# harvardinformatics/IMCoalHMM

Hardware: AMD Instinct MI355X
Metric: alignment columns/sec (forward pass), 20-state isolation HMM (higher is better)
Workload: dtype f64

## Files before the change

### imcoalhmm_amd/csrc/imcoal_fwd.hip

```cpp
#include <hip/hip_runtime.h>

#include <algorithm>
#include <cerrno>
#include <climits>
#include <cmath>
#include <cstdint>
#include <cstdio>
#include <cstdlib>
#include <cstring>
#include <list>
#include <atomic>
#include <chrono>
#include <map>
#include <set>
#include <memory>
#include <mutex>
#include <condition_variable>
#include <string>
#include <vector>

#include <unistd.h>

#include "../../include/imcoal_fwd.h"
#include "kernels_plain.hpp"
// ... 82 lines not shown
    uint64_t next_obs_id = 1, next_dict_id = 1;
    size_t seg_override = 0;
    int compression = 1;
    int kernel_pref = 0;
    bool profile = false;
    bool rank1_handoff = true;
    int blocked_variant = 4;
    int wide_blocked = -1;
    int z4_stream = -1;
    bool table_pairs = true;
    int table_triples = -1;
    bool table_split = true;
    int table_split_max = -1;
    bool xcd_affine = true;
    int fuse_tail = 1;
    bool fuse_head = true;
    bool pack_table = true;
    bool guard = false;
    bool use_graphs = false;
    std::vector<Ev3> events;
    std::map<int, std::shared_ptr<DictDev>> dicts;
    uint64_t last_plan[8] = {0, 0, 0, 0, 0, 0, 0, 0};
    uint64_t r1_checked = 0, r1_collapsed = 0;
    std::string last_kernels;
    std::vector<const void *> lds_opted;
} g;

void drop_plans();
void model_release();

// ... 19 lines not shown
    if (std::strncmp(prop.gcnArchName, "gfx950", 6) != 0)
        return fail(IMC_ERR_NODEVICE, std::string("device is ") + prop.gcnArchName + ", this library is built for gfx950 only");
    g.cus = prop.multiProcessorCount > 0 ? prop.multiProcessorCount : 256;
    HIP_TRY(hipStreamCreateWithFlags(&g.stream, hipStreamNonBlocking));
    g.use_graphs = std::getenv("IMC_GRAPH") != nullptr;
    if (const char *gd = std::getenv("IMC_GUARD")) g.guard = std::atoi(gd) != 0;
    if (const char *bv = std::getenv("IMC_BLOCKED")) { const int v = std::atoi(bv); if (v >= 2 && v <= 5) g.blocked_variant = v; }
    if (const char *r1 = std::getenv("IMC_RANK1")) g.rank1_handoff = std::atoi(r1) != 0;
    if (const char *pt = std::getenv("IMC_PACK_TABLE")) g.pack_table = std::atoi(pt) != 0;
    if (const char *tp = std::getenv("IMC_TABLE_PAIRS")) g.table_pairs = std::atoi(tp) != 0;
    if (const char *fh = std::getenv("IMC_FUSE_HEAD")) g.fuse_head = std::atoi(fh) != 0;
    if (const char *ts = std::getenv("IMC_TABLE_SPLIT")) g.table_split = std::atoi(ts) != 0;
    if (const char *tm = std::getenv("IMC_TABLE_SPLIT_MAX")) g.table_split_max = std::max(0, std::atoi(tm));
    if (const char *tt = std::getenv("IMC_TABLE_TRIPLES")) g.table_triples = std::atoi(tt) != 0 ? 1 : 0;
    if (const char *ft = std::getenv("IMC_FUSE_TAIL")) g.fuse_tail = std::max(0, std::min(2, std::atoi(ft)));
    if (const char *xa = std::getenv("IMC_XCD_AFFINE")) g.xcd_affine = std::atoi(xa) != 0;
    if (const char *wb = std::getenv("IMC_WIDE_BLOCKED")) { const int v = std::atoi(wb); if (v >= -1 && v <= 1) g.wide_blocked = v; }
    if (const char *zs = std::getenv("IMC_Z4_STREAM")) { const int v = std::atoi(zs); if (v >= -1 && v <= 1) g.z4_stream = v; }
    g.pid = me;
    g.ready = true;
    return IMC_OK;
}

struct GuardRec { hipDeviceptr_t va; size_t va_size; hipMemGenericAllocationHandle_t handle; hipDeviceptr_t map; size_t map_size; };
std::map<void *, GuardRec> &g_guard = *new std::map<void *, GuardRec>();

hipError_t dev_alloc(void **p, size_t bytes)
{
    bytes = std::max<size_t>(bytes, 16);
    if (!g.guard) return hipMalloc(p, bytes);
// ... 224 lines not shown
    if (zipped) {
        if (int rc = install_encoding(o, dd, enc)) {
            obs_release(o);
            delete o;
            return rc;
        }
    }
    *out = o;
    return IMC_OK;
}


using ChainFn = void (*)(const ChainDesc *, int, const uint32_t *, uint32_t, uint32_t, const double *, const int *,
                         const int *, uint32_t, double *, int *, double *, int);

struct KernelChoice {
    int R = 0, G = 0, NP = 0, VPW = 0, minw = 1;
    void (*plain)(PropArgs) = nullptr;
    void (*zip)(PropArgs) = nullptr;
    size_t (*zip_lds)(int) = nullptr;
    ChainFn chain = nullptr;
    void (*big_table_raw)(BigArgs) = nullptr;
    void (*big_table_level)(BigArgs, const uint16_t *, int) = nullptr;
    void (*big_prop)(BigArgs, const BigBlock *) = nullptr;
    int big_prop_waves = 0;
    void (*big_vec)(BigArgs, const BigBlock *, int, int) = nullptr;
    void (*big_vec_tail)(BigArgs, const BigBlock *, int, int) = nullptr;
    int big_vec_waves = 0;
    int big_nslab = 0;
    size_t big_lds = 0;
    void (*zip2)(BigArgs) = nullptr;
    size_t (*zip2_lds)(int) = nullptr;
    void (*zip3)(BigArgs) = nullptr;
    size_t (*zip3_lds)(int) = nullptr;
    void (*zip4)(BigArgs) = nullptr;
    void (*zip4w)(BigArgs) = nullptr;
// ... 16 lines not shown
    bool chain_self_emax = false;
    bool use3() const;
    size_t blocked_lds(int A) const { return use3() ? zip3_lds(A) : zip2_lds(A); }
};

template <int R, int G, int MW>
KernelChoice make_kc()
{
    constexpr int NP = R * G;
    KernelChoice k;
    k.R = R; k.G = G; k.NP = NP; k.VPW = 64 / G; k.minw = MW;
    k.plain = k_propagate<R, G, MW>;
    k.zip = k_zpropagate<R, G>;
    k.zip_lds = &ZipGeom<R, G>::lds_bytes;
    k.chain = k_chain<NP, (NP <= 12 ? 6 : NP <= 24 ? 4 : NP <= 32 ? 3 : NP <= 64 ? 2 : 1)>;
    k.chain_self_emax = true;
    if constexpr (NP % 4 == 0 && NP <= 24) {
        k.zip2 = k_zpropagate2<NP / 4>;
        k.zip2_lds = &Zip2Geom<NP / 4>::lds_bytes;
        k.zip3 = k_zpropagate3<NP / 4>;
        k.zip3_lds = &Zip3Geom<NP / 4>::lds_bytes;
        k.tok_doubles = Zip3Geom<NP / 4>::TOK;
        if constexpr (NP <= 24) {
            k.zip4 = k_zpropagate4<NP / 4, false, true>;
            k.zip4w = k_zpropagate4<NP / 4, true, true>;
            k.zip4s = k_zpropagate4<NP / 4, false, false>;
            k.zip4sw = k_zpropagate4<NP / 4, true, false>;
            k.zip4_raw = k_z4_raw<NP / 4>;
            k.zip4_level = k_z4_level<NP / 4>;
            k.zip4_level2 = k_z4_level2<NP / 4, false>;
// ... 134 lines not shown

struct Plan {
    std::vector<uint64_t> key;
    KernelChoice *kc = nullptr;
    bool wide = false;
    int N = 0, S = 0, B = 0, n_chunks = 0;
    uint32_t n_segs = 0, n_vecs = 0;
    std::vector<Group> groups;
    size_t pstride = 0;
    SegDesc *d_segs = nullptr;
    VecDesc *d_vecs = nullptr;
    std::vector<Level> levels;
    int32_t *d_final_vec = nullptr;
    uint64_t chain_steps = 0;
    bool finish_fused = false;
    double *d_params = nullptr, *d_out = nullptr;
    double *h_params[2] = {nullptr, nullptr};
    hipEvent_t ev_params[2] = {nullptr, nullptr};
    bool ev_used[2] = {false, false};
    int slot = 0;
    double *h_out = nullptr;
    double *h_out_dev = nullptr;
    double *h_params_dev[2] = {nullptr, nullptr};
    hipStream_t last_stream = nullptr;
    int last_slot = 0;
    bool have_last = false;
    bool busy = false;
    hipGraphExec_t graph = nullptr;
    uint64_t calls = 0;
    uint64_t lp[8] = {0, 0, 0, 0, 0, 0, 0, 0};
    std::string kernels;
    void release()
    {
        if (graph) (void)hipGraphExecDestroy(graph);
        dev_free(d_segs); dev_free(d_vecs); dev_free(d_final_vec);
        for (auto &l : levels) l.release();
        for (auto &gr : groups) { dev_free(gr.d_seg_ids); dev_free(gr.d_seg_out); dev_free(gr.d_blocks); dev_free(gr.d_hot); dev_free(gr.d_tab_desc); dev_free(gr.d_tab_desc2); dev_free(gr.d_tab_desc3); dev_free(gr.d_tails); dev_free(gr.d_tailX); dev_free(gr.d_tailE); dev_free(gr.d_tail_arrive); dev_free(gr.d_tab_order); dev_free(gr.d_tab_lvl); dev_free(gr.d_big_blocks); dev_free(gr.d_Ctab); dev_free(gr.d_Cpack); dev_free(gr.d_cex); dev_free(gr.d_tail_blocks); dev_free(gr.d_r1flag); dev_free(gr.d_r1at); dev_free(gr.d_r1u); dev_free(gr.d_r1alpha); }
        dev_free(d_params); dev_free(d_out);
        for (int k = 0; k < 2; ++k) { (void)hipHostFree(h_params[k]); if (ev_params[k]) (void)hipEventDestroy(ev_params[k]); }
        (void)hipHostFree(h_out);
    }
};

std::list<std::unique_ptr<Plan>> g_plans;
constexpr size_t MAX_PLANS = 4;

void wait_all_idle(std::unique_lock<std::mutex> &lk)
{
    g_cv.wait(lk, [] {
        for (auto &p : g_plans)
// ... 85 lines not shown
    int n_chunks = 0, N = 0, S = 0, B = 0;
    bool op_mode = false;
    KernelChoice *kc = nullptr;
    bool wide = false, wide_ok = true;
    bool mfma() const { return kc->use3() || wide; }
    std::unique_ptr<Plan> p;
    bool big = false;
    std::vector<int> chunk_group;
    std::vector<SegDesc> segs;
    std::vector<uint8_t> seg_first;
    std::vector<uint32_t> chunk_seg;
    std::vector<VecDesc> vecs;
    std::vector<std::vector<std::pair<uint32_t, uint32_t>>> chunk_units;
    std::vector<uint32_t> chunk_unit, unit_vec0;
    std::vector<uint8_t> unit_first;
    struct HostLevel { std::vector<uint32_t> chunk_seg, vec0; std::vector<uint8_t> first; std::vector<ChainDesc> chains; uint32_t n_vecs; };
    std::vector<HostLevel> hl;
    std::vector<int32_t> final_vec;

    static bool z4_streamed(double tables_bytes, int n_sets)
    {
        if (g.z4_stream >= 0) return g.z4_stream == 1;
        return (g.xcd_affine && n_sets > 1) || tables_bytes <= Z4_STREAM_MAX_BYTES;
    }

    size_t handoff_head(const Group &gr) const
    {
        double cols = 0.0, toks = 0.0;
        for (int f : gr.chunks) { cols += (double)chunks[f]->L; toks += (double)(gr.zip ? chunks[f]->ntok[gr.level] : chunks[f]->L); }
        const double span = toks > 0.0 ? cols / toks : 1.0;
        return round_up(std::max<size_t>(R1_MIN_HEAD, (size_t)(R1_HEAD_COLUMNS / span)), 16);
    }

// ... 367 lines not shown
                else
                    for (Z2Block &bk : gr.blocks)
                        if (bk.first == 2) bk.first = 1;
            }
        }
        if (vecs.size() >= (size_t)UINT32_MAX / 2) return fail(IMC_ERR_ARG, "too many vectors in one call");
        p->n_segs = (uint32_t)segs.size();
        p->n_vecs = (uint32_t)vecs.size();
        p->pstride = round_up((size_t)kc->NP + (size_t)kc->NP * kc->NP + (size_t)S * kc->NP, 2);

        return IMC_OK;
    }

    void make_hierarchy()
    {
        hl.assign(1, HostLevel());
        hl[0].chunk_seg = chunk_unit; hl[0].vec0 = unit_vec0; hl[0].first = unit_first; hl[0].n_vecs = p->n_vecs;
        for (;;) {
            const HostLevel &cur = hl.back();
            uint32_t kmax = 0;
            for (int f = 0; f < n_chunks; ++f) kmax = std::max(kmax, cur.chunk_seg[f + 1] - cur.chunk_seg[f]);
            if (kmax <= 1 && hl.size() > 1) break;
            if (kmax == 0) break;
            const uint32_t gsz = kmax <= 16 ? kmax : std::max<uint32_t>(12, (uint32_t)std::ceil(std::cbrt((double)kmax)));
            p->chain_steps += gsz;
            HostLevel nx;
            nx.chunk_seg.assign(n_chunks + 1, 0);
            nx.n_vecs = 0;
            for (int f = 0; f < n_chunks; ++f) {
                nx.chunk_seg[f] = (uint32_t)nx.vec0.size();
                const uint32_t s0 = cur.chunk_seg[f], s1 = cur.chunk_seg[f + 1];
                for (uint32_t rb = s0; rb < s1; rb += gsz) {
                    const uint32_t re = std::min(rb + gsz, s1);
                    const bool fst = rb == s0 && !op_mode;
                    nx.vec0.push_back(nx.n_vecs);
                    nx.first.push_back(fst);
                    const int nvv = fst ? 1 : N;
                    for (int c = 0; c < nvv; ++c) nx.chains.push_back(ChainDesc{rb, re, (uint32_t)c, nx.n_vecs + c, fst ? 1u : 0u, 0u});
                    nx.n_vecs += nvv;
                }
            }
            nx.chunk_seg[n_chunks] = (uint32_t)nx.vec0.size();
            const bool done = kmax <= gsz;
            hl.push_back(std::move(nx));
            if (done) break;
        }
        final_vec.assign(std::max(n_chunks, 1), -1);
        bool all_from_chains = hl.size() > 1 && !op_mode && n_chunks > 0;
        for (int f = 0; f < n_chunks; ++f) {
            const HostLevel &last = hl.back();
            if (last.chunk_seg[f + 1] > last.chunk_seg[f]) final_vec[f] = (int32_t)last.vec0[last.chunk_seg[f]];
            else all_from_chains = false;
        }
        p->finish_fused = false;
        if (all_from_chains) {
            HostLevel &last = hl.back();
            std::vector<char> seen((size_t)n_chunks, 0);
            for (ChainDesc &cd : last.chains)
                for (int f = 0; f < n_chunks; ++f)
                    if (cd.first && final_vec[f] == (int32_t)cd.out_vec) { cd.chunk1 = (uint32_t)f + 1; seen[f] = 1; }
            p->finish_fused = std::all_of(seen.begin(), seen.end(), [](char c) { return c != 0; });
            if (!p->finish_fused)
                for (ChainDesc &cd : last.chains) cd.chunk1 = 0;
        }

    }

    int upload(Plan **out)
    {
        while (g_plans.size() >= MAX_PLANS) {
            auto victim = g_plans.end();
            for (auto it = g_plans.begin(); it != g_plans.end(); ++it)
                if (!(*it)->busy) victim = it;
            if (victim == g_plans.end()) break;
            (*victim)->release();
            g_plans.erase(victim);
        }

        Plan *q = p.get();
        auto up = [&](void **d, const void *h, size_t bytes) -> hipError_t {
// ... 12 lines not shown
        if (e == hipSuccess) e = up((void **)&q->d_vecs, vecs.data(), vecs.size() * sizeof(VecDesc));
        if (e == hipSuccess) e = up((void **)&q->d_final_vec, final_vec.data(), final_vec.size() * 4);
        q->levels.resize(hl.size());
        for (size_t l = 0; l < hl.size() && e == hipSuccess; ++l) {
            Level &lv = q->levels[l];
            lv.n_segs = (uint32_t)hl[l].vec0.size();
            lv.n_vecs = hl[l].n_vecs;
            lv.n_chains = (uint32_t)hl[l].chains.size();
            const size_t nv = std::max<size_t>(lv.n_vecs, 1), ns = std::max<size_t>(lv.n_segs, 1);
            e = up((void **)&lv.d_vec0, hl[l].vec0.data(), hl[l].vec0.size() * 4);
            if (e == hipSuccess) e = up((void **)&lv.d_first, hl[l].first.data(), hl[l].first.size());
            if (e == hipSuccess) e = up((void **)&lv.d_chains, hl[l].chains.data(), hl[l].chains.size() * sizeof(ChainDesc));
            if (e == hipSuccess) e = zalloc((void **)&lv.d_P, (size_t)B * nv * kc->NP * 8);
            if (e == hipSuccess) e = zalloc((void **)&lv.d_EX, (size_t)B * nv * 4);
            if (e == hipSuccess) e = zalloc((void **)&lv.d_EMAX, (size_t)B * ns * 4);
        }
        for (Group &gr : q->groups) {
            if (gr.zip2 && e == hipSuccess) e = up((void **)&gr.d_blocks, gr.blocks.data(), gr.blocks.size() * sizeof(Z2Block));
            if (!gr.tails.empty() && e == hipSuccess) {
                const size_t slots = (size_t)B * n_chunks * gr.tail_stride;
                e = up((void **)&gr.d_tails, gr.tails.data(), gr.tails.size() * sizeof(Z2Tail));
                if (e == hipSuccess) e = dev_alloc((void **)&gr.d_tailX, slots * kc->tok_doubles * 8);
                if (e == hipSuccess) e = dev_alloc((void **)&gr.d_tailE, slots * 128);
                if (e == hipSuccess) e = zalloc((void **)&gr.d_tail_arrive, (size_t)B * n_chunks * 4);
            }
            if (gr.zip4 && e == hipSuccess) {
                std::vector<uint64_t> cnt((size_t)gr.A, 0);
                for (int f : gr.chunks)
                    for (size_t z = 0; z < chunks[f]->tok_count[gr.level].size() && z < cnt.size(); ++z) cnt[z] += chunks[f]->tok_count[gr.level][z];
                const std::vector<uint16_t> ids = imc::hot_order(cnt);
// ... 56 lines not shown
        if (e == hipSuccess) e = hipHostGetDevicePointer((void **)&q->h_out_dev, q->h_out, 0);
        if (e != hipSuccess) {
            q->release();
            return fail(e == hipErrorOutOfMemory ? IMC_ERR_OOM : IMC_ERR_HIP,
                        std::string("plan allocation: ") + hipGetErrorString(e));
        }
        g_plans.push_front(std::move(p));
        *out = q;
        return IMC_OK;
    }
};

int build_plan(const imc_obs *const *chunks, int n_chunks, int N, int S, int B, bool op_mode, Plan **out)
{
    std::vector<uint64_t> key;
    key.reserve(n_chunks + 5);
    for (int f = 0; f < n_chunks; ++f) key.push_back(chunks[f]->id);
    key.push_back((uint64_t)N); key.push_back((uint64_t)S); key.push_back((uint64_t)B);
    key.push_back((uint64_t)g.seg_override); key.push_back((uint64_t)(g.compression * 4 + g.kernel_pref + (op_mode ? 64 : 0) + g.blocked_variant * 128 + (g.z4_stream + 1) * 1024 + (g.wide_blocked + 1) * 4096));
    { const char *fl = std::getenv("IMC_FORCE_LEVEL"); key.push_back(fl ? (uint64_t)(std::atoi(fl) + 1) : 0u); }
    for (auto it = g_plans.begin(); it != g_plans.end(); ++it) {
        if ((*it)->key == key) {
            g_plans.splice(g_plans.begin(), g_plans, it);
            *out = g_plans.front().get();
            return IMC_OK;
        }
    }
    bool prefer_gemm = g.kernel_pref == 2;
    if (g.kernel_pref == 0 && N > 24 && N <= 64 && n_chunks > 0) {
        double total = 0.0;
        for (int f = 0; f < n_chunks; ++f) total += (double)chunks[f]->L;
        bool tokens = g.compression != 0;
        for (int f = 0; f < n_chunks; ++f) tokens = tokens && chunks[f]->dict && chunks[f]->nsym == S;
        prefer_gemm = total >= 1.0e6 && total / n_chunks >= 5.0e3 && (tokens || N > 40);
    }
// ... 394 lines not shown
    const size_t lds = ((size_t)WPB * kc->VPW * kc->NP + (size_t)p->S * kc->NP) * 8;
    if (lds > LDS_BUDGET) return fail(IMC_ERR_ARG, "emission table (S x N) too large for LDS");
    if (lds > 48 * 1024)
        if (int rc = allow_lds_budget(kc->plain)) return rc;
    hipLaunchKernelGGL(kc->plain, grid, dim3(WPB * 64), lds, stream, prop_args(p, gr));
    note("k_propagate<" + std::to_string(kc->R) + "," + std::to_string(kc->G) + ">" + stream_tag(gr));
    account(gr);
    HIP_TRY(hipGetLastError());
    return IMC_OK;
}


int Launch::stitch() const
{
    const int N = p->N, NP = kc->NP;
    for (size_t l = 0; l + 1 < p->levels.size(); ++l) {
        const Level &in = p->levels[l], &ot = p->levels[l + 1];
        if (!in.n_segs || !ot.n_chains) continue;
        if (!kc->chain_self_emax) {
            hipLaunchKernelGGL(k_emax, dim3((in.n_segs + 255) / 256, (unsigned)B), dim3(256), 0, stream,
                               in.d_vec0, in.d_first, in.n_segs, in.n_vecs, N, in.d_EX, in.d_EMAX);
            HIP_TRY(hipGetLastError());
        }
        const int threads = (int)round_up((size_t)NP, 64);
        const bool last_level = l + 2 == p->levels.size();
        hipLaunchKernelGGL(kc->chain, dim3(ot.n_chains, (unsigned)B), dim3(threads), 0, stream,
                           ot.d_chains, N, in.d_vec0, in.n_segs, in.n_vecs, in.d_P, in.d_EX, in.d_EMAX,
                           ot.n_vecs, ot.d_P, ot.d_EX, (last_level && p->finish_fused) ? out : (double *)nullptr, p->n_chunks);
        HIP_TRY(hipGetLastError());
    }
    if (p->n_chunks && !p->finish_fused) {
        const Level &last = p->levels.back();
        hipLaunchKernelGGL(k_finish, dim3((p->n_chunks + 63) / 64, (unsigned)B), dim3(64), 0, stream,
                           p->d_final_vec, p->n_chunks, N, NP, last.n_vecs, last.d_P, last.d_EX, out);
        HIP_TRY(hipGetLastError());
    }
    return IMC_OK;
}

int enqueue(Plan *p, hipStream_t stream, double *out, bool allow_tail = true)
{
    hipStreamCaptureStatus cap = hipStreamCaptureStatusNone;
    (void)hipStreamIsCapturing(stream, &cap);
    if (cap == hipStreamCaptureStatusNone && p->have_last && p->last_stream != stream)
        HIP_TRY(hipStreamWaitEvent(stream, p->ev_params[p->last_slot], 0));
// ... 21 lines not shown
    if (L.tail_used) L.note("fused-tail");
    if (!L.tail_used)
        if (int rc = L.stitch()) return rc;
    if (L.prof) {
        HIP_TRY(hipEventRecord(L.ev.c, stream));
        g.events.push_back(L.ev);
    }
    if (cap == hipStreamCaptureStatusNone) {
        HIP_TRY(hipEventRecord(p->ev_params[p->slot], stream));
        p->ev_used[p->slot] = true;
        p->last_stream = stream;
        p->last_slot = p->slot;
        p->have_last = true;
    }
    return IMC_OK;
}

void collect_rank1_stats(Plan *p)
{
    g.r1_checked = g.r1_collapsed = 0;
    for (Group &gr : p->groups) {
        if (!gr.rank1 || gr.r1_segs.empty() || gr.checkpoints.empty()) continue;
        std::vector<int> flags((size_t)p->B * p->n_segs);
        if (hipMemcpy(flags.data(), gr.d_r1flag, flags.size() * 4, hipMemcpyDeviceToHost) != hipSuccess) continue;
        for (int b = 0; b < p->B; ++b)
            for (const auto &sl : gr.r1_segs) {
                if ((int)sl.second <= gr.checkpoints[0]) continue;
                ++g.r1_checked;
                g.r1_collapsed += flags[(size_t)b * p->n_segs + sl.first] ? 1 : 0;
            }
// ... 46 lines not shown
        explicit Busy(Plan *q) : p(q) { p->busy = true; }
        ~Busy() { p->busy = false; g_cv.notify_all(); }
    } busy(p);
    const auto h1 = now();
    if (int rc = stage_params(p, pis, Ts, Es, g.use_graphs)) return rc;
    const size_t n_out = (size_t)B * n_chunks;
    for (size_t k = 0; k < n_out; ++k) reinterpret_cast<volatile uint64_t *>(p->h_out)[k] = OUT_SENTINEL;
    std::atomic_thread_fence(std::memory_order_release);
    const auto h2 = now();
    const bool use_graph = !g.profile && g.use_graphs && p->calls >= 1;
    if (use_graph && !p->graph) {
        hipGraph_t gr = nullptr;
        HIP_TRY(hipStreamBeginCapture(g.stream, hipStreamCaptureModeThreadLocal));
        const int rc = enqueue(p, g.stream, p->h_out_dev);
        const hipError_t ec = hipStreamEndCapture(g.stream, &gr);
        if (rc) { if (gr) (void)hipGraphDestroy(gr); return rc; }
        if (ec != hipSuccess) return fail(IMC_ERR_HIP, std::string("hipStreamEndCapture: ") + hipGetErrorString(ec));
        const hipError_t ei = hipGraphInstantiate(&p->graph, gr, nullptr, nullptr, 0);
        (void)hipGraphDestroy(gr);
        if (ei != hipSuccess) { p->graph = nullptr; return fail(IMC_ERR_HIP, std::string("hipGraphInstantiate: ") + hipGetErrorString(ei)); }
    }
    if (use_graph) HIP_TRY(hipGraphLaunch(p->graph, g.stream));
    else if (int rc = enqueue(p, g.stream, p->h_out_dev)) return rc;
    ++p->calls;
    for (int k = 0; k < 8; ++k) g.last_plan[k] = p->lp[k];
    g.last_kernels = p->kernels;
    const auto h3 = now();
    const hipStream_t st = g.stream;
    lk.unlock();
    const hipError_t ew = n_out ? wait_results(st, p->h_out, n_out) : hipStreamSynchronize(st);
    lk.lock();
    HIP_TRY(ew);
    const auto h4 = now();
    collect_rank1_stats(p);
    if (dbg_host) {
        auto us = [](auto a, auto b) { return std::chrono::duration<double, std::micro>(b - a).count(); };
        static double acc[5] = {0, 0, 0, 0, 0};
        static int n_acc = 0;
        acc[0] += us(h0, h1); acc[1] += us(h1, h2); acc[2] += us(h2, h3); acc[3] += us(h3, h4); acc[4] += us(h4, now());
        if (++n_acc % 20 == 0) {
            fprintf(stderr, "[imc] host us per call: check+plan %.1f  stage %.1f  enqueue %.1f  sync wait %.1f  stats %.1f\n",
                    acc[0] / 20, acc[1] / 20, acc[2] / 20, acc[3] / 20, acc[4] / 20);
            for (double &a : acc) a = 0.0;
        }
    }
    for (int b = 0; b < B; ++b) {
// ... 9 lines not shown
}

int run_state(const imc_obs *const *chunks, int n_chunks, bool op_mode, int B, int N, int S, const double *pis,
              const double *Ts, const double *Es, double *out_state, int *out_exp)
{
    std::lock_guard<std::mutex> lk(g_mu);
    if (int rc = ensure_ctx()) return rc;
    if (int rc = check_args(chunks, n_chunks, B, N, S, pis, Ts, Es)) return rc;
    if (!out_state || !out_exp) return fail(IMC_ERR_ARG, "output buffer is null");
    for (int f = 0; f < n_chunks; ++f)
        if (chunks[f]->L == 0) return fail(IMC_ERR_ARG, "imc_forward_state: empty chunk");
    HIP_TRY(hipSetDevice(g.device));
    Plan *p = nullptr;
    if (int rc = build_plan(chunks, n_chunks, N, S, B, op_mode, &p)) return rc;
    if (int rc = stage_params(p, pis, Ts, Es, g.use_graphs)) return rc;
    if (int rc = enqueue(p, g.stream, p->d_out, false)) return rc;
    ++p->calls;
    for (int k = 0; k < 8; ++k) g.last_plan[k] = p->lp[k];
    g.last_kernels = p->kernels;
    const size_t per = op_mode ? (size_t)N * N : (size_t)N, pere = op_mode ? (size_t)N : 1;
    const size_t n_state = (size_t)B * n_chunks * per, n_exp = (size_t)B * n_chunks * pere;
    double *d_state = nullptr;
    int *d_exp = nullptr;
    hipError_t e = dev_alloc((void **)&d_state, std::max<size_t>(n_state * 8, 16));
    if (e == hipSuccess) e = dev_alloc((void **)&d_exp, std::max<size_t>(n_exp * 4, 16));
    if (e == hipSuccess) {
        const Level &last = p->levels.back();
        hipLaunchKernelGGL(k_export, dim3((unsigned)n_chunks, (unsigned)B), dim3(256), 0, g.stream, p->d_final_vec, n_chunks, N,
                           p->kc->NP, last.n_vecs, last.d_P, last.d_EX, op_mode ? 1 : 0, d_state, d_exp);
        e = hipGetLastError();
    }
// ... 627 lines not shown
    return run_batch(chunks, n_chunks, B, N, S, pis, Ts, Es, nullptr, out_per_chunk);
}

int imc_forward_batch_device(const imc_obs *const *chunks, int n_chunks, int B, int N, int S, const double *pis,
                             const double *Ts, const double *Es, double *d_out_partial, void *hip_stream)
{
    if (!d_out_partial) return fail(IMC_ERR_ARG, "d_out_partial is null");
    std::lock_guard<std::mutex> lk(g_mu);
    if (int rc = ensure_ctx()) return rc;
    if (int rc = check_args(chunks, n_chunks, B, N, S, pis, Ts, Es)) return rc;
    HIP_TRY(hipSetDevice(g.device));
    hipStream_t st = (hipStream_t)hip_stream;
    Plan *p = nullptr;
    if (int rc = build_plan(chunks, n_chunks, N, S, B, false, &p)) return rc;
    if (int rc = stage_params(p, pis, Ts, Es, g.use_graphs)) return rc;
    if (int rc = enqueue(p, st, p->d_out)) return rc;
    ++p->calls;
    for (int k = 0; k < 8; ++k) g.last_plan[k] = p->lp[k];
    g.last_kernels = p->kernels;
    hipLaunchKernelGGL(k_sum_chunks, dim3((B + 63) / 64), dim3(64), 0, st, p->d_out, n_chunks, B, d_out_partial);
    HIP_TRY(hipGetLastError());
    return IMC_OK;
}

int imc_set_segment_length(size_t columns)
{
    std::lock_guard<std::mutex> lk(g_mu);
    g.seg_override = columns;
    return IMC_OK;
}

// ... 181 lines not shown
```

### imcoalhmm_amd/csrc/kernels_stitch.hpp

```cpp
#pragma once
#include "kernels_plain.hpp"

struct ChainDesc {
    uint32_t seg_begin, seg_end;
    uint32_t c;
    uint32_t out_vec;
    uint32_t first;
    uint32_t chunk1;
};

__global__ void k_emax(const uint32_t *seg_vec0, const uint8_t *seg_first, uint32_t n_segs, uint32_t n_vecs, int N,
                       const int *EX, int *EMAX)
{
    const uint32_t s = blockIdx.x * blockDim.x + threadIdx.x;
    const int b = blockIdx.y;
    if (s >= n_segs) return;
    const int *e = EX + (size_t)b * n_vecs + seg_vec0[s];
    int m = e[0];
    if (!seg_first[s])
        for (int c = 1; c < N; ++c) m = max(m, e[c]);
    EMAX[(size_t)b * n_segs + s] = m;
}

template <int NP, int D>
// ... 111 lines not shown
    int e = 0;
    (void)frexp(tot, &e);
    e = (tot > 0.0 && tot < INFINITY) ? e : 0;
    const size_t gv = (size_t)b * out_n_vecs + cd.out_vec;
    if (mine) {
        double *dst = cd.first ? Pout + gv * NP + i : Pout + (gv - cd.c) * NP + (size_t)i * NP + cd.c;
        *dst = ldexp(a, -e);
    }
    if (i == 0) {
        EXout[gv] = etot + e;
        if (fin_out && cd.chunk1)
            fin_out[(size_t)b * n_chunks + (cd.chunk1 - 1)] = (double)(etot + e) * 0.693147180559945309417232121458 + log(ldexp(tot, -e));
    }
}

__global__ void k_finish(const int32_t *final_vec, int n_chunks, int N, int NP, uint32_t n_vecs, const double *P,
                         const int *EX, double *out)
{
    const int f = blockIdx.x * blockDim.x + threadIdx.x;
    const int b = blockIdx.y;
    if (f >= n_chunks) return;
    const int32_t v = final_vec[f];
    double r = 0.0;
    if (v >= 0) {
        const double *p = P + ((size_t)b * n_vecs + v) * NP;
        double tot = 0.0;
        for (int c = 0; c < N; ++c) tot += p[c];
        r = (double)EX[(size_t)b * n_vecs + v] * 0.693147180559945309417232121458 + log(tot);
    }
    out[(size_t)b * n_chunks + f] = r;
// ... 40 lines not shown
```

### imcoalhmm_amd/csrc/plan_host.hpp

```cpp
#pragma once

#include <algorithm>
#include <cstdint>
#include <utility>
#include <vector>

#include "pair_dict.hpp"

namespace imc {

struct alignas(16) Desc4 { int32_t x, y, z, w; };
static_assert(sizeof(Desc4) == 16 && alignof(Desc4) == 16, "Desc4 is one 16-byte load");

struct TableSchedule {
    std::vector<Desc4> desc;
    std::vector<std::pair<int, int>> launches;
};

inline std::vector<tok_t> dict_order(const PairDict &d, const std::vector<int> &depth)
{
    std::vector<tok_t> order;
    for (int z = d.nsym; z < d.alphabet; ++z) order.push_back((tok_t)z);
    std::stable_sort(order.begin(), order.end(), [&](tok_t x, tok_t y) { return depth[x] < depth[y]; });
    return order;
// ... 160 lines not shown
    PhaseTable t;
    int first = 0, wg = 0;
    auto phase = [&](int sets, int n_sets_total) {
        t.ph_begin[t.n_phases] = wg; t.ph_first[t.n_phases] = first; t.ph_sets[t.n_phases] = sets;
        ++t.n_phases;
        wg += sets >= 8 ? 8 * blocks * (n_sets_total / 8) : 8 * ((blocks + 8 / sets - 1) / (8 / sets));
        first += n_sets_total;
    };
    if (B >= 8) phase(8, B / 8 * 8);
    for (int sets : {4, 2, 1})
        if ((B % 8) & sets) phase(sets, sets);
    t.grid = wg;
    return t;
}

}
```

Measured before the change: 394.3 billion.

## Add fast wave-level chain stitch kernel and fuse last chain level via arrival counters

Adds a new chain-stitching kernel that runs on a single wavefront. It broadcasts weights with readlane and prefetches D steps of packed double2 rows. When the hierarchy qualifies, it also fuses the final chain level into the previous one: each chain publishes its result to a global slot, and the last-arriving wavefront, chosen by an atomic ticket counter, performs the final reduction. This removes one kernel launch and the separate emax pass. The cost is atomic and fence overhead, extra device buffers, and counter reset handling on error paths.

```diff
diff --git a/imcoalhmm_amd/csrc/imcoal_fwd.hip b/imcoalhmm_amd/csrc/imcoal_fwd.hip
--- a/imcoalhmm_amd/csrc/imcoal_fwd.hip
+++ b/imcoalhmm_amd/csrc/imcoal_fwd.hip
@@ -120,6 +120,8 @@
     int table_split_max = -1;
     bool xcd_affine = true;
     int fuse_tail = 1;
+    bool chain_fast = true;
+    int chain_group = 0;
     bool fuse_head = true;
     bool pack_table = true;
     bool guard = false;
@@ -169,6 +171,8 @@
     if (const char *tm = std::getenv("IMC_TABLE_SPLIT_MAX")) g.table_split_max = std::max(0, std::atoi(tm));
     if (const char *tt = std::getenv("IMC_TABLE_TRIPLES")) g.table_triples = std::atoi(tt) != 0 ? 1 : 0;
     if (const char *ft = std::getenv("IMC_FUSE_TAIL")) g.fuse_tail = std::max(0, std::min(2, std::atoi(ft)));
+    if (const char *cf = std::getenv("IMC_CHAIN_FAST")) g.chain_fast = std::atoi(cf) != 0;
+    if (const char *cg = std::getenv("IMC_CHAIN_GROUP")) { const int v = std::atoi(cg); if (v >= 2) g.chain_group = v; }
     if (const char *xa = std::getenv("IMC_XCD_AFFINE")) g.xcd_affine = std::atoi(xa) != 0;
     if (const char *wb = std::getenv("IMC_WIDE_BLOCKED")) { const int v = std::atoi(wb); if (v >= -1 && v <= 1) g.wide_blocked = v; }
     if (const char *zs = std::getenv("IMC_Z4_STREAM")) { const int v = std::atoi(zs); if (v >= -1 && v <= 1) g.z4_stream = v; }
@@ -423,12 +427,17 @@
 using ChainFn = void (*)(const ChainDesc *, int, const uint32_t *, uint32_t, uint32_t, const double *, const int *,
                          const int *, uint32_t, double *, int *, double *, int);
 
+using ChainFastFn = void (*)(const ChainDesc *, int, uint32_t, const double *, const int *, uint32_t, double *, int *, double *,
+                             int, ChainFuse);
+
 struct KernelChoice {
     int R = 0, G = 0, NP = 0, VPW = 0, minw = 1;
     void (*plain)(PropArgs) = nullptr;
     void (*zip)(PropArgs) = nullptr;
     size_t (*zip_lds)(int) = nullptr;
     ChainFn chain = nullptr;
+    ChainFastFn chain_fast = nullptr;
+    ChainFastFn chain_fast_fused = nullptr;
     void (*big_table_raw)(BigArgs) = nullptr;
     void (*big_table_level)(BigArgs, const uint16_t *, int) = nullptr;
     void (*big_prop)(BigArgs, const BigBlock *) = nullptr;
@@ -475,6 +484,10 @@
     k.zip = k_zpropagate<R, G>;
     k.zip_lds = &ZipGeom<R, G>::lds_bytes;
     k.chain = k_chain<NP, (NP <= 12 ? 6 : NP <= 24 ? 4 : NP <= 32 ? 3 : NP <= 64 ? 2 : 1)>;
+    if constexpr (NP <= 32 && NP % 2 == 0) {
+        k.chain_fast = k_chain_fast<NP, (NP <= 12 ? 6 : NP <= 24 ? 4 : 3), false>;
+        k.chain_fast_fused = k_chain_fast<NP, (NP <= 12 ? 6 : NP <= 24 ? 4 : 3), true>;
+    }
     k.chain_self_emax = true;
     if constexpr (NP % 4 == 0 && NP <= 24) {
         k.zip2 = k_zpropagate2<NP / 4>;
@@ -639,6 +652,12 @@
     int32_t *d_final_vec = nullptr;
     uint64_t chain_steps = 0;
     bool finish_fused = false;
+    bool last_fused = false;
+    ChainFinal *d_finals = nullptr;
+    double *d_chain_pub = nullptr;
+    int *d_chain_arrive = nullptr;
+    uint32_t n_finals = 0, n_chain_slots = 0;
+    size_t chain_arrive_bytes = 0;
     double *d_params = nullptr, *d_out = nullptr;
     double *h_params[2] = {nullptr, nullptr};
     hipEvent_t ev_params[2] = {nullptr, nullptr};
@@ -659,6 +678,7 @@
     {
         if (graph) (void)hipGraphExecDestroy(graph);
         dev_free(d_segs); dev_free(d_vecs); dev_free(d_final_vec);
+        dev_free(d_finals); dev_free(d_chain_pub); dev_free(d_chain_arrive);
         for (auto &l : levels) l.release();
         for (auto &gr : groups) { dev_free(gr.d_seg_ids); dev_free(gr.d_seg_out); dev_free(gr.d_blocks); dev_free(gr.d_hot); dev_free(gr.d_tab_desc); dev_free(gr.d_tab_desc2); dev_free(gr.d_tab_desc3); dev_free(gr.d_tails); dev_free(gr.d_tailX); dev_free(gr.d_tailE); dev_free(gr.d_tail_arrive); dev_free(gr.d_tab_order); dev_free(gr.d_tab_lvl); dev_free(gr.d_big_blocks); dev_free(gr.d_Ctab); dev_free(gr.d_Cpack); dev_free(gr.d_cex); dev_free(gr.d_tail_blocks); dev_free(gr.d_r1flag); dev_free(gr.d_r1at); dev_free(gr.d_r1u); dev_free(gr.d_r1alpha); }
         dev_free(d_params); dev_free(d_out);
@@ -774,9 +794,10 @@
     std::vector<std::vector<std::pair<uint32_t, uint32_t>>> chunk_units;
     std::vector<uint32_t> chunk_unit, unit_vec0;
     std::vector<uint8_t> unit_first;
-    struct HostLevel { std::vector<uint32_t> chunk_seg, vec0; std::vector<uint8_t> first; std::vector<ChainDesc> chains; uint32_t n_vecs; };
+    using HostLevel = imc::ChainLevel;
     std::vector<HostLevel> hl;
     std::vector<int32_t> final_vec;
+    std::vector<ChainFinal> finals;
 
     static bool z4_streamed(double tables_bytes, int n_sets)
     {
@@ -1174,56 +1195,18 @@
 
     void make_hierarchy()
     {
-        hl.assign(1, HostLevel());
-        hl[0].chunk_seg = chunk_unit; hl[0].vec0 = unit_vec0; hl[0].first = unit_first; hl[0].n_vecs = p->n_vecs;
-        for (;;) {
-            const HostLevel &cur = hl.back();
-            uint32_t kmax = 0;
-            for (int f = 0; f < n_chunks; ++f) kmax = std::max(kmax, cur.chunk_seg[f + 1] - cur.chunk_seg[f]);
-            if (kmax <= 1 && hl.size() > 1) break;
-            if (kmax == 0) break;
-            const uint32_t gsz = kmax <= 16 ? kmax : std::max<uint32_t>(12, (uint32_t)std::ceil(std::cbrt((double)kmax)));
-            p->chain_steps += gsz;
-            HostLevel nx;
-            nx.chunk_seg.assign(n_chunks + 1, 0);
-            nx.n_vecs = 0;
-            for (int f = 0; f < n_chunks; ++f) {
-                nx.chunk_seg[f] = (uint32_t)nx.vec0.size();
-                const uint32_t s0 = cur.chunk_seg[f], s1 = cur.chunk_seg[f + 1];
-                for (uint32_t rb = s0; rb < s1; rb += gsz) {
-                    const uint32_t re = std::min(rb + gsz, s1);
-                    const bool fst = rb == s0 && !op_mode;
-                    nx.vec0.push_back(nx.n_vecs);
-                    nx.first.push_back(fst);
-                    const int nvv = fst ? 1 : N;
-                    for (int c = 0; c < nvv; ++c) nx.chains.push_back(ChainDesc{rb, re, (uint32_t)c, nx.n_vecs + c, fst ? 1u : 0u, 0u});
-                    nx.n_vecs += nvv;
-                }
-            }
-            nx.chunk_seg[n_chunks] = (uint32_t)nx.vec0.size();
-            const bool done = kmax <= gsz;
-            hl.push_back(std::move(nx));
-            if (done) break;
-        }
-        final_vec.assign(std::max(n_chunks, 1), -1);
-        bool all_from_chains = hl.size() > 1 && !op_mode && n_chunks > 0;
-        for (int f = 0; f < n_chunks; ++f) {
-            const HostLevel &last = hl.back();
-            if (last.chunk_seg[f + 1] > last.chunk_seg[f]) final_vec[f] = (int32_t)last.vec0[last.chunk_seg[f]];
-            else all_from_chains = false;
-        }
-        p->finish_fused = false;
-        if (all_from_chains) {
-            HostLevel &last = hl.back();
-            std::vector<char> seen((size_t)n_chunks, 0);
-            for (ChainDesc &cd : last.chains)
-                for (int f = 0; f < n_chunks; ++f)
-                    if (cd.first && final_vec[f] == (int32_t)cd.out_vec) { cd.chunk1 = (uint32_t)f + 1; seen[f] = 1; }
-            p->finish_fused = std::all_of(seen.begin(), seen.end(), [](char c) { return c != 0; });
-            if (!p->finish_fused)
-                for (ChainDesc &cd : last.chains) cd.chunk1 = 0;
-        }
-
+        HostLevel l0;
+        l0.chunk_seg = chunk_unit; l0.vec0 = unit_vec0; l0.first = unit_first; l0.n_vecs = p->n_vecs;
+        imc::ChainHierarchy h = imc::build_hierarchy(std::move(l0), n_chunks, N, op_mode, (uint32_t)g.chain_group,
+                                                     g.chain_fast && kc->chain_fast != nullptr);
+        hl = std::move(h.levels);
+        final_vec = std::move(h.final_vec);
+        finals = std::move(h.finals);
+        p->chain_steps += h.chain_steps;
+        p->finish_fused = h.finish_fused;
+        p->last_fused = h.last_fused;
+        p->n_finals = (uint32_t)finals.size();
+        p->n_chain_slots = h.n_slots;
     }
 
     int upload(Plan **out)
@@ -1266,6 +1249,12 @@
             if (e == hipSuccess) e = zalloc((void **)&lv.d_P, (size_t)B * nv * kc->NP * 8);
             if (e == hipSuccess) e = zalloc((void **)&lv.d_EX, (size_t)B * nv * 4);
             if (e == hipSuccess) e = zalloc((void **)&lv.d_EMAX, (size_t)B * ns * 4);
+        }
+        if (q->last_fused && e == hipSuccess) {
+            q->chain_arrive_bytes = (size_t)B * q->n_finals * CHAIN_CTR_STRIDE * 4;
+            e = up((void **)&q->d_finals, finals.data(), finals.size() * sizeof(ChainFinal));
+            if (e == hipSuccess) e = zalloc((void **)&q->d_chain_pub, (size_t)B * q->n_chain_slots * chain_slot_doubles(kc->NP) * 8);
+            if (e == hipSuccess) e = zalloc((void **)&q->d_chain_arrive, q->chain_arrive_bytes);
         }
         for (Group &gr : q->groups) {
             if (gr.zip2 && e == hipSuccess) e = up((void **)&gr.d_blocks, gr.blocks.data(), gr.blocks.size() * sizeof(Z2Block));
@@ -1352,11 +1341,12 @@
 int build_plan(const imc_obs *const *chunks, int n_chunks, int N, int S, int B, bool op_mode, Plan **out)
 {
     std::vector<uint64_t> key;
-    key.reserve(n_chunks + 5);
+    key.reserve(n_chunks + 7);
     for (int f = 0; f < n_chunks; ++f) key.push_back(chunks[f]->id);
     key.push_back((uint64_t)N); key.push_back((uint64_t)S); key.push_back((uint64_t)B);
     key.push_back((uint64_t)g.seg_override); key.push_back((uint64_t)(g.compression * 4 + g.kernel_pref + (op_mode ? 64 : 0) + g.blocked_variant * 128 + (g.z4_stream + 1) * 1024 + (g.wide_blocked + 1) * 4096));
     { const char *fl = std::getenv("IMC_FORCE_LEVEL"); key.push_back(fl ? (uint64_t)(std::atoi(fl) + 1) : 0u); }
+    key.push_back((uint64_t)g.chain_group);
     for (auto it = g_plans.begin(); it != g_plans.end(); ++it) {
         if ((*it)->key == key) {
             g_plans.splice(g_plans.begin(), g_plans, it);
@@ -1781,21 +1771,36 @@
 int Launch::stitch() const
 {
     const int N = p->N, NP = kc->NP;
-    for (size_t l = 0; l + 1 < p->levels.size(); ++l) {
+    const bool fast = g.chain_fast && kc->chain_fast != nullptr;
+    const size_t n_launch = p->levels.size() - 1 - (p->last_fused ? 1 : 0);
+    for (size_t l = 0; l < n_launch; ++l) {
         const Level &in = p->levels[l], &ot = p->levels[l + 1];
         if (!in.n_segs || !ot.n_chains) continue;
+        const bool last_level = l + 1 == n_launch;
+        double *fin_out = (last_level && p->finish_fused) ? out : (double *)nullptr;
+        if (fast) {
+            ChainFuse fz{};
+            if (last_level && p->last_fused) {
+                const Level &fl = p->levels.back();
+                fz = ChainFuse{p->d_finals, p->d_chain_pub, p->d_chain_arrive, p->n_chain_slots, p->n_finals, fl.n_vecs, fl.d_P, fl.d_EX};
+            }
+            hipLaunchKernelGGL(fz.fin ? kc->chain_fast_fused : kc->chain_fast, dim3(ot.n_chains, (unsigned)B), dim3(64), 0, stream,
+                               ot.d_chains, N, in.n_vecs, in.d_P, in.d_EX, ot.n_vecs, ot.d_P, ot.d_EX, fin_out, p->n_chunks, fz);
+            HIP_TRY(hipGetLastError());
+            continue;
+        }
         if (!kc->chain_self_emax) {
             hipLaunchKernelGGL(k_emax, dim3((in.n_segs + 255) / 256, (unsigned)B), dim3(256), 0, stream,
                                in.d_vec0, in.d_first, in.n_segs, in.n_vecs, N, in.d_EX, in.d_EMAX);
             HIP_TRY(hipGetLastError());
         }
         const int threads = (int)round_up((size_t)NP, 64);
-        const bool last_level = l + 2 == p->levels.size();
         hipLaunchKernelGGL(kc->chain, dim3(ot.n_chains, (unsigned)B), dim3(threads), 0, stream,
                            ot.d_chains, N, in.d_vec0, in.n_segs, in.n_vecs, in.d_P, in.d_EX, in.d_EMAX,
-                           ot.n_vecs, ot.d_P, ot.d_EX, (last_level && p->finish_fused) ? out : (double *)nullptr, p->n_chunks);
+                           ot.n_vecs, ot.d_P, ot.d_EX, fin_out, p->n_chunks);
         HIP_TRY(hipGetLastError());
     }
+    if (p->last_fused) note("chain-fused<" + std::to_string(p->levels.size() - 1) + ">");
     if (p->n_chunks && !p->finish_fused) {
         const Level &last = p->levels.back();
         hipLaunchKernelGGL(k_finish, dim3((p->n_chunks + 63) / 64, (unsigned)B), dim3(64), 0, stream,
@@ -1847,6 +1852,14 @@
         p->have_last = true;
     }
     return IMC_OK;
+}
+
+void reset_chain_counters(Plan *p, hipStream_t stream)
+{
+    if (!p->d_chain_arrive) return;
+    (void)hipStreamSynchronize(stream);
+    (void)hipMemset(p->d_chain_arrive, 0, p->chain_arrive_bytes);
+    (void)hipGetLastError();
 }
 
 void collect_rank1_stats(Plan *p)
@@ -1923,14 +1936,14 @@
         HIP_TRY(hipStreamBeginCapture(g.stream, hipStreamCaptureModeThreadLocal));
         const int rc = enqueue(p, g.stream, p->h_out_dev);
         const hipError_t ec = hipStreamEndCapture(g.stream, &gr);
-        if (rc) { if (gr) (void)hipGraphDestroy(gr); return rc; }
+        if (rc) { if (gr) (void)hipGraphDestroy(gr); reset_chain_counters(p, g.stream); return rc; }
         if (ec != hipSuccess) return fail(IMC_ERR_HIP, std::string("hipStreamEndCapture: ") + hipGetErrorString(ec));
         const hipError_t ei = hipGraphInstantiate(&p->graph, gr, nullptr, nullptr, 0);
         (void)hipGraphDestroy(gr);
         if (ei != hipSuccess) { p->graph = nullptr; return fail(IMC_ERR_HIP, std::string("hipGraphInstantiate: ") + hipGetErrorString(ei)); }
     }
     if (use_graph) HIP_TRY(hipGraphLaunch(p->graph, g.stream));
-    else if (int rc = enqueue(p, g.stream, p->h_out_dev)) return rc;
+    else if (int rc = enqueue(p, g.stream, p->h_out_dev)) { reset_chain_counters(p, g.stream); return rc; }
     ++p->calls;
     for (int k = 0; k < 8; ++k) g.last_plan[k] = p->lp[k];
     g.last_kernels = p->kernels;
@@ -1939,6 +1952,7 @@
     lk.unlock();
     const hipError_t ew = n_out ? wait_results(st, p->h_out, n_out) : hipStreamSynchronize(st);
     lk.lock();
+    if (ew != hipSuccess) reset_chain_counters(p, st);
     HIP_TRY(ew);
     const auto h4 = now();
     collect_rank1_stats(p);
@@ -1978,7 +1992,7 @@
     Plan *p = nullptr;
     if (int rc = build_plan(chunks, n_chunks, N, S, B, op_mode, &p)) return rc;
     if (int rc = stage_params(p, pis, Ts, Es, g.use_graphs)) return rc;
-    if (int rc = enqueue(p, g.stream, p->d_out, false)) return rc;
+    if (int rc = enqueue(p, g.stream, p->d_out, false)) { reset_chain_counters(p, g.stream); return rc; }
     ++p->calls;
     for (int k = 0; k < 8; ++k) g.last_plan[k] = p->lp[k];
     g.last_kernels = p->kernels;
@@ -2636,7 +2650,7 @@
     Plan *p = nullptr;
     if (int rc = build_plan(chunks, n_chunks, N, S, B, false, &p)) return rc;
     if (int rc = stage_params(p, pis, Ts, Es, g.use_graphs)) return rc;
-    if (int rc = enqueue(p, st, p->d_out)) return rc;
+    if (int rc = enqueue(p, st, p->d_out)) { reset_chain_counters(p, st); return rc; }
     ++p->calls;
     for (int k = 0; k < 8; ++k) g.last_plan[k] = p->lp[k];
     g.last_kernels = p->kernels;
diff --git a/imcoalhmm_amd/csrc/kernels_stitch.hpp b/imcoalhmm_amd/csrc/kernels_stitch.hpp
--- a/imcoalhmm_amd/csrc/kernels_stitch.hpp
+++ b/imcoalhmm_amd/csrc/kernels_stitch.hpp
@@ -1,13 +1,11 @@
 #pragma once
 #include "kernels_plain.hpp"
-
-struct ChainDesc {
-    uint32_t seg_begin, seg_end;
-    uint32_t c;
-    uint32_t out_vec;
-    uint32_t first;
-    uint32_t chunk1;
-};
+#include "plan_host.hpp"
+
+using imc::ChainDesc;
+using imc::ChainFinal;
+using imc::CHAIN_CTR_STRIDE;
+using imc::chain_slot_doubles;
 
 __global__ void k_emax(const uint32_t *seg_vec0, const uint8_t *seg_first, uint32_t n_segs, uint32_t n_vecs, int N,
                        const int *EX, int *EMAX)
@@ -149,6 +147,165 @@
     }
 }
 
+template <int NP>
+__device__ __forceinline__ void chain_step_fast(double &a, int &etot, const double2 (&cur)[NP / 2], int ex, bool mine)
+{
+    const int ex0 = __builtin_amdgcn_readfirstlane(ex);
+    int em = ex0;
+    if (__builtin_amdgcn_ballot_w64(ex != ex0) != 0) em = wave_max_i32_dpp(ex);
+    const double wv = mine ? ldexp(a, ex - em) : 0.0;
+    int e = wave_max_i32_dpp(wv != 0.0 ? __builtin_amdgcn_frexp_exp(wv) : INT_MIN);
+    e = e == INT_MIN ? 0 : e;
+    const int lo = __double2loint(wv), hi = __double2hiint(wv);
+    double acc0 = 0.0, acc1 = 0.0;
+#pragma unroll
+    for (int m = 0; m < NP / 2; ++m) {
+        const double wx = __hiloint2double(__builtin_amdgcn_readlane(hi, 2 * m), __builtin_amdgcn_readlane(lo, 2 * m));
+        const double wy = __hiloint2double(__builtin_amdgcn_readlane(hi, 2 * m + 1), __builtin_amdgcn_readlane(lo, 2 * m + 1));
+        acc0 = fma(cur[m].x, wx, acc0);
+        acc1 = fma(cur[m].y, wy, acc1);
+    }
+    a = mine ? ldexp(acc0 + acc1, -e) : 0.0;
+    etot += em + e;
+}
+
+template <int NP, int D, class Fetch>
+__device__ __forceinline__ void chain_run_fast(double &a, int &etot, int nsteps, bool mine, Fetch fetch)
+{
+    double2 pk[D][NP / 2];
+    int exr[D];
+#pragma unroll
+    for (int s = 0; s < D; ++s)
+        if (s < nsteps) fetch(s, pk[s], exr[s]);
+    for (int t0 = 0; t0 < nsteps; t0 += D) {
+#pragma unroll
+        for (int s = 0; s < D; ++s) {
+            const int t = t0 + s;
+            if (t < nsteps) {
+                double2 cur[NP / 2];
+#pragma unroll
+                for (int m = 0; m < NP / 2; ++m) cur[m] = pk[s][m];
+                const int ex = exr[s];
+                if (t + D < nsteps) fetch(t + D, pk[s], exr[s]);
+                chain_step_fast<NP>(a, etot, cur, ex, mine);
+            }
+        }
+    }
+}
+
+template <int NP>
+__device__ __forceinline__ void chain_normalise(double &a, int &etot, double &tot)
+{
+    const int lo = __double2loint(a), hi = __double2hiint(a);
+    tot = 0.0;
+#pragma unroll
+    for (int c = 0; c < NP; ++c) tot += __hiloint2double(__builtin_amdgcn_readlane(hi, c), __builtin_amdgcn_readlane(lo, c));
+    int e = 0;
+    (void)frexp(tot, &e);
+    e = (tot > 0.0 && tot < INFINITY) ? e : 0;
+    a = ldexp(a, -e);
+    etot += e;
+    tot = ldexp(tot, -e);
+}
+
+struct ChainFuse {
+    const ChainFinal *fin;
+    double *pub;
+    int *arrive;
+    uint32_t n_slots, n_fin;
+    uint32_t fin_n_vecs;
+    double *finP;
+    int *finEX;
+};
+
+template <int NP, int D, bool FUSE>
+__global__ __launch_bounds__(64) void k_chain_fast(
+    const ChainDesc *chains, int N, uint32_t in_n_vecs, const double *Pin, const int *EXin,
+    uint32_t out_n_vecs, double *Pout, int *EXout, double *fin_out, int n_chunks, ChainFuse fz)
+{
+    static_assert(NP <= 32 && D > 0 && NP % 2 == 0, "one wavefront, register ring, the vector in scalar registers");
+    constexpr int SLOT = chain_slot_doubles(NP);
+    constexpr double LN2 = 0.693147180559945309417232121458;
+    const ChainDesc cd = chains[blockIdx.x];
+    const int b = blockIdx.y, i = threadIdx.x;
+    const double *Pb = Pin + (size_t)b * in_n_vecs * NP;
+    const int *EXb = EXin + (size_t)b * in_n_vecs;
+    const bool mine = i < N;
+    const int ii = mine ? i : 0;
+
+    double a;
+    int etot;
+    if (cd.first) {
+        a = mine ? Pb[(size_t)cd.vfirst * NP + i] : 0.0;
+        etot = EXb[cd.vfirst];
+    } else {
+        a = (i == (int)cd.c) ? 1.0 : 0.0;
+        etot = 0;
+    }
+    const int nsteps = (int)cd.seg_end - (int)cd.seg_begin - (cd.first ? 1 : 0);
+    chain_run_fast<NP, D>(a, etot, nsteps, mine, [&](int t, double2 (&row)[NP / 2], int &ex) {
+        const size_t v0 = (size_t)cd.vbase + (size_t)t * N;
+        ex = EXb[v0 + ii];
+        const double2 *src = reinterpret_cast<const double2 *>(Pb + (v0 + ii) * NP);
+#pragma unroll
+        for (int m = 0; m < NP / 2; ++m) row[m] = src[m];
+    });
+    double tot;
+    chain_normalise<NP>(a, etot, tot);
+
+    if (!FUSE || !cd.fin1) {
+        const size_t gv = (size_t)b * out_n_vecs + cd.out_vec;
+        if (mine) {
+            double *dst = cd.first ? Pout + gv * NP + i : Pout + (gv - cd.c) * NP + (size_t)i * NP + cd.c;
+            *dst = a;
+        }
+        if (i == 0) {
+            EXout[gv] = etot;
+            if (fin_out && cd.chunk1) fin_out[(size_t)b * n_chunks + (cd.chunk1 - 1)] = (double)etot * LN2 + log(tot);
+        }
+        return;
+    }
+    if constexpr (FUSE) {
+    const ChainFinal cf = fz.fin[cd.fin1 - 1];
+    double *pubb = fz.pub + (size_t)b * fz.n_slots * SLOT;
+    if (cf.n_arrive > 1) {
+        double *slot = pubb + (size_t)cd.pub * SLOT;
+        if (mine) __hip_atomic_store(&slot[i], a, __ATOMIC_RELAXED, __HIP_MEMORY_SCOPE_AGENT);
+        if (i == 0) __hip_atomic_store(reinterpret_cast<int *>(slot + NP), etot, __ATOMIC_RELAXED, __HIP_MEMORY_SCOPE_AGENT);
+        asm volatile("s_waitcnt vmcnt(0)" ::: "memory");
+        int *ctr = fz.arrive + ((size_t)b * fz.n_fin + (cd.fin1 - 1)) * CHAIN_CTR_STRIDE;
+        int ticket = 0;
+        if (i == 0) ticket = __hip_atomic_fetch_add(ctr, 1, __ATOMIC_RELAXED, __HIP_MEMORY_SCOPE_AGENT);
+        ticket = __builtin_amdgcn_readfirstlane(ticket);
+        if (ticket != (int)cf.n_arrive - 1) return;
+        __builtin_amdgcn_fence(__ATOMIC_ACQUIRE, "wavefront");
+        if (i == 0) __hip_atomic_store(ctr, 0, __ATOMIC_RELAXED, __HIP_MEMORY_SCOPE_AGENT);
+        const double *s0 = pubb + (size_t)cf.slot0 * SLOT;
+        const double v = __hip_atomic_load(&s0[ii], __ATOMIC_RELAXED, __HIP_MEMORY_SCOPE_AGENT);
+        a = mine ? v : 0.0;
+        etot = __hip_atomic_load(reinterpret_cast<const int *>(s0 + NP), __ATOMIC_RELAXED, __HIP_MEMORY_SCOPE_AGENT);
+    }
+    chain_run_fast<NP, D>(a, etot, (int)cf.nsteps, mine, [&](int t, double2 (&row)[NP / 2], int &ex) {
+        const double *u = pubb + ((size_t)cf.slot0 + 1 + (size_t)t * N) * SLOT;
+        ex = __hip_atomic_load(reinterpret_cast<const int *>(u + (size_t)ii * SLOT + NP), __ATOMIC_RELAXED, __HIP_MEMORY_SCOPE_AGENT);
+#pragma unroll
+        for (int m = 0; m < NP / 2; ++m) {
+            const int c0 = 2 * m, c1 = 2 * m + 1;
+            const double x = __hip_atomic_load(&u[(size_t)(c0 < N ? c0 : 0) * SLOT + ii], __ATOMIC_RELAXED, __HIP_MEMORY_SCOPE_AGENT);
+            const double y = __hip_atomic_load(&u[(size_t)(c1 < N ? c1 : 0) * SLOT + ii], __ATOMIC_RELAXED, __HIP_MEMORY_SCOPE_AGENT);
+            row[m] = make_double2(c0 < N ? x : 0.0, c1 < N ? y : 0.0);
+        }
+    });
+    chain_normalise<NP>(a, etot, tot);
+    const size_t gv = (size_t)b * fz.fin_n_vecs + cf.out_vec;
+    if (mine) fz.finP[gv * NP + i] = a;
+    if (i == 0) {
+        fz.finEX[gv] = etot;
+        if (fin_out && cf.chunk1) fin_out[(size_t)b * n_chunks + (cf.chunk1 - 1)] = (double)etot * LN2 + log(tot);
+    }
+    }
+}
+
 __global__ void k_finish(const int32_t *final_vec, int n_chunks, int N, int NP, uint32_t n_vecs, const double *P,
                          const int *EX, double *out)
 {
diff --git a/imcoalhmm_amd/csrc/plan_host.hpp b/imcoalhmm_amd/csrc/plan_host.hpp
--- a/imcoalhmm_amd/csrc/plan_host.hpp
+++ b/imcoalhmm_amd/csrc/plan_host.hpp
@@ -1,6 +1,7 @@
 #pragma once
 
 #include <algorithm>
+#include <cmath>
 #include <cstdint>
 #include <utility>
 #include <vector>
@@ -198,4 +199,153 @@
     return t;
 }
 
-}
+
+struct ChainDesc {
+    uint32_t seg_begin, seg_end;
+    uint32_t c;
+    uint32_t out_vec;
+    uint32_t first;
+    uint32_t chunk1;
+    uint32_t vbase;
+    uint32_t vfirst;
+    uint32_t fin1, pub;
+    uint32_t pad[2];
+};
+static_assert(sizeof(ChainDesc) == 48, "ChainDesc is three 16-byte loads");
+
+struct ChainFinal {
+    uint32_t n_arrive;
+    uint32_t slot0;
+    uint32_t nsteps;
+    uint32_t out_vec;
+    uint32_t chunk1;
+    uint32_t pad[3];
+};
+static_assert(sizeof(ChainFinal) == 32, "ChainFinal is two 16-byte loads");
+
+constexpr int CHAIN_CTR_STRIDE = 32;
+constexpr int chain_slot_doubles(int NP) { return (NP * 8 + 4 + 127) / 128 * 16; }
+
+constexpr uint32_t CHAIN_FUSE_MAX_STEPS = 16;
+
+struct ChainLevel {
+    std::vector<uint32_t> chunk_seg, vec0;
+    std::vector<uint8_t> first;
+    std::vector<ChainDesc> chains;
+    uint32_t n_vecs = 0;
+};
+
+struct ChainHierarchy {
+    std::vector<ChainLevel> levels;
+    std::vector<int32_t> final_vec;
+    uint64_t chain_steps = 0;
+    bool finish_fused = false;
+    bool last_fused = false;
+    std::vector<ChainFinal> finals;
+    uint32_t n_slots = 0;
+};
+
+inline ChainHierarchy build_hierarchy(ChainLevel level0, int n_chunks, int N, bool op_mode, uint32_t group, bool fuse)
+{
+    ChainHierarchy h;
+    h.levels.push_back(std::move(level0));
+    for (;;) {
+        const ChainLevel &cur = h.levels.back();
+        uint32_t kmax = 0;
+        for (int f = 0; f < n_chunks; ++f) kmax = std::max(kmax, cur.chunk_seg[f + 1] - cur.chunk_seg[f]);
+        if (kmax <= 1 && h.levels.size() > 1) break;
+        if (kmax == 0) break;
+        uint32_t gsz;
+        if (group >= 2) gsz = std::min(kmax, group);
+        else gsz = kmax <= 16 ? kmax : std::max<uint32_t>(12, (uint32_t)std::ceil(std::cbrt((double)kmax)));
+        h.chain_steps += gsz;
+        ChainLevel nx;
+        nx.chunk_seg.assign((size_t)n_chunks + 1, 0);
+        nx.n_vecs = 0;
+        for (int f = 0; f < n_chunks; ++f) {
+            nx.chunk_seg[f] = (uint32_t)nx.vec0.size();
+            const uint32_t s0 = cur.chunk_seg[f], s1 = cur.chunk_seg[f + 1];
+            for (uint32_t rb = s0; rb < s1; rb += gsz) {
+                const uint32_t re = std::min(rb + gsz, s1);
+                const bool fst = rb == s0 && !op_mode;
+                nx.vec0.push_back(nx.n_vecs);
+                nx.first.push_back(fst);
+                const int nvv = fst ? 1 : N;
+                const uint32_t k0 = rb + (fst ? 1u : 0u);
+                for (int c = 0; c < nvv; ++c) {
+                    ChainDesc cd{};
+                    cd.seg_begin = rb; cd.seg_end = re; cd.c = (uint32_t)c; cd.out_vec = nx.n_vecs + c; cd.first = fst ? 1u : 0u;
+                    cd.vbase = k0 < re ? cur.vec0[k0] : 0u;
+                    cd.vfirst = fst ? cur.vec0[rb] : 0u;
+                    nx.chains.push_back(cd);
+                }
+                nx.n_vecs += nvv;
+            }
+        }
+        nx.chunk_seg[n_chunks] = (uint32_t)nx.vec0.size();
+        const bool done = kmax <= gsz;
+        h.levels.push_back(std::move(nx));
+        if (done) break;
+    }
+    h.final_vec.assign((size_t)std::max(n_chunks, 1), -1);
+    bool all_from_chains = h.levels.size() > 1 && !op_mode && n_chunks > 0;
+    for (int f = 0; f < n_chunks; ++f) {
+        const ChainLevel &last = h.levels.back();
+        if (last.chunk_seg[f + 1] > last.chunk_seg[f]) h.final_vec[f] = (int32_t)last.vec0[last.chunk_seg[f]];
+        else all_from_chains = false;
+    }
+    if (all_from_chains) {
+        ChainLevel &last = h.levels.back();
+        std::vector<char> seen((size_t)n_chunks, 0);
+        for (ChainDesc &cd : last.chains)
+            for (int f = 0; f < n_chunks; ++f)
+                if (cd.first && h.final_vec[f] == (int32_t)cd.out_vec) { cd.chunk1 = (uint32_t)f + 1; seen[f] = 1; }
+        h.finish_fused = std::all_of(seen.begin(), seen.end(), [](char c) { return c != 0; });
+        if (!h.finish_fused)
+            for (ChainDesc &cd : last.chains) cd.chunk1 = 0;
+    }
+    if (!fuse || op_mode || h.levels.size() < 3) return h;
+    const ChainLevel &last = h.levels.back();
+    ChainLevel &prev = h.levels[h.levels.size() - 2];
+    std::vector<ChainFinal> finals;
+    std::vector<uint32_t> seg_slot(prev.vec0.size(), 0), seg_fin(prev.vec0.size(), 0);
+    uint32_t n_slots = 0;
+    size_t n_last_chains = 0;
+    for (int f = 0; f < n_chunks; ++f) {
+        const uint32_t l0 = last.chunk_seg[f], l1 = last.chunk_seg[f + 1];
+        const uint32_t s0 = prev.chunk_seg[f], s1 = prev.chunk_seg[f + 1];
+        if (l1 == l0 && s1 == s0) continue;
+        if (l1 - l0 != 1 || s1 == s0 || !last.first[l0] || !prev.first[s0] || s1 - s0 - 1 > CHAIN_FUSE_MAX_STEPS) return h;
+        const ChainDesc *fc = n_last_chains < last.chains.size() ? &last.chains[n_last_chains++] : nullptr;
+        if (!fc || !fc->first || fc->seg_begin != s0 || fc->seg_end != s1 || fc->out_vec != last.vec0[l0]) return h;
+        ChainFinal cf{};
+        cf.slot0 = n_slots; cf.nsteps = s1 - s0 - 1; cf.n_arrive = 1 + cf.nsteps * (uint32_t)N;
+        cf.out_vec = fc->out_vec; cf.chunk1 = fc->chunk1;
+        for (uint32_t s = s0; s < s1; ++s) {
+            if (s > s0 && prev.first[s]) return h;
+            seg_slot[s] = n_slots; seg_fin[s] = (uint32_t)finals.size() + 1;
+            n_slots += s == s0 ? 1u : (uint32_t)N;
+        }
+        finals.push_back(cf);
+    }
+    if (finals.empty() || n_last_chains != last.chains.size()) return h;
+    size_t ci = 0;
+    for (size_t s = 0; s < prev.vec0.size(); ++s) {
+        const uint32_t n = prev.first[s] ? 1u : (uint32_t)N;
+        for (uint32_t c = 0; c < n; ++c, ++ci) {
+            if (ci >= prev.chains.size() || prev.chains[ci].out_vec != prev.vec0[s] + c || !seg_fin[s]) return h;
+        }
+    }
+    if (ci != prev.chains.size()) return h;
+    ci = 0;
+    for (size_t s = 0; s < prev.vec0.size(); ++s) {
+        const uint32_t n = prev.first[s] ? 1u : (uint32_t)N;
+        for (uint32_t c = 0; c < n; ++c, ++ci) { prev.chains[ci].fin1 = seg_fin[s]; prev.chains[ci].pub = seg_slot[s] + c; }
+    }
+    h.last_fused = true;
+    h.finals = std::move(finals);
+    h.n_slots = n_slots;
+    return h;
+}
+
+}
```

Result: no change. 395.7 billion, median of 2 (+0.4%).
